# kirilllzaitsev/vision_mtl

Measured on AMD Instinct MI355X. Metric: images/sec fwd+bwd, basic model 128x256, higher is better.
Workload: dtype f32

## Files before the change

vision_mtl_amd/csrc/conv_igemm.hip:

```cpp
#include <mutex>
#include <unordered_map>

#include "common.h"

#define BK 32
#define LDT BK

struct ConvP {
  const float* x = nullptr;
  const float* wp = nullptr;
  const float* bias = nullptr;
  float* y = nullptr;
  float* stats = nullptr;
  int B = 0, H = 0, W = 0, Cs = 0;
  int Ho = 0, Wo = 0, ldy = 0;
  int Nw = 0;
  int Cout = 0;
  int KH = 0, KW = 0, stride = 0, pad = 0;
  int Ktot = 0, M = 0;
  int act = 0;
  int shuffle = 0;
  int tiles_m = 0, tiles_n = 0;
  const float* x2 = nullptr;
  int C2s = 0;
  int ksplit = 1, ksteps_per_split = 0;
  const float* ez_x = nullptr;
  const float* ez_mean = nullptr;
  const float* ez_invstd = nullptr;
  const float* ez_gamma = nullptr;
  const float* ez_beta = nullptr;
  int ez_act = 0;
};

__device__ __attribute__((aligned(16))) float g_zero_page[4] = {0.f, 0.f, 0.f, 0.f};

template <int N>
__device__ __forceinline__ void wait_vmcnt() {
  asm volatile("s_waitcnt vmcnt(%0)" ::"n"(N) : "memory");
}

__device__ __forceinline__ void glds16(const float* src, float* lds_dst) {
  __builtin_amdgcn_global_load_lds((const __attribute__((address_space(1))) void*)src,
                                   (__attribute__((address_space(3))) void*)lds_dst, 16, 0, 0);
}


__device__ __forceinline__ void split3(f32x4 v, u32x2& p1, u32x2& p2, u32x2& p3) {
  unsigned x[4], r1[4], r2[4];
#pragma unroll
  for (int e = 0; e < 4; ++e) {
    x[e] = __float_as_uint(v[e]);
    const float f1 = v[e] - __uint_as_float(x[e] & 0xFFFF0000u);
    r1[e] = __float_as_uint(f1);
    const float f2 = f1 - __uint_as_float(r1[e] & 0xFFFF0000u);
    r2[e] = __float_as_uint(f2);
  }
  p1 = (u32x2){__builtin_amdgcn_perm(x[1], x[0], 0x07060302u), __builtin_amdgcn_perm(x[3], x[2], 0x07060302u)};
  p2 = (u32x2){__builtin_amdgcn_perm(r1[1], r1[0], 0x07060302u), __builtin_amdgcn_perm(r1[3], r1[2], 0x07060302u)};
  p3 = (u32x2){__builtin_amdgcn_perm(r2[1], r2[0], 0x07060302u), __builtin_amdgcn_perm(r2[3], r2[2], 0x07060302u)};
}

template <int TM, int TN, int WAVES_M, int WAVES_N, bool UP2 = false, int NT = 0, int NS = 0, int PL = 0>
__global__ __launch_bounds__(256, (TM * TN >= 20 && WAVES_N == 2) ? 2 : 1) void conv_igemm_kernel(ConvP p) {
  constexpr int BM = WAVES_M * TM * 16;
  constexpr int BNM = WAVES_N * TN * 16;
  constexpr int BN = BNM + NT;
  constexpr int RA = (BM + 31) / 32;
  constexpr int RB = (BN + 31) / 32;
  constexpr int NBUF = NS >= 2 ? NS : 2;
  constexpr int BNR = NS >= 2 ? RB * 32 : BN;
  static_assert(WAVES_M * WAVES_N == 4, "4 waves per workgroup");
  static_assert(NT == 0 || WAVES_N == 1, "tail columns need all waves to span the full tile width");
  static_assert(NS == 0 || (NS >= 2 && NS <= 4 && BM % 32 == 0), "LDS-DMA staging: 2..4 buffers, whole 32-row passes");
  static_assert(PL == 0 || PL == 1 || PL == 3, "operand planes: fp32, bf16 or bf16x3");
  static_assert(PL == 0 || (NS == 0 && (NT == 0 || PL == 1)), "bf16 operands: register staging; bf16x3: no tail columns");

  extern __shared__ __attribute__((aligned(16))) float smem[];
  float* As = smem;
  float* Bs = smem + NBUF * BM * LDT;

  const int tid = threadIdx.x;
  const int lane = tid & 63;
  const int wv = tid >> 6;
  const int wm = wv / WAVES_N, wn = wv % WAVES_N;
  const int l15 = lane & 15, lq = lane >> 4;

  const int nwg = p.tiles_m * p.tiles_n;
  const int bid = xcd_remap(blockIdx.x, nwg);
  const int tile_m = bid / p.tiles_n, tile_n = bid % p.tiles_n;
  const int n0 = tile_n * BN;
  const int tiles_q = UP2 ? p.tiles_m >> 2 : p.tiles_m;
  const int phase = UP2 ? tile_m / tiles_q : 0;
  const int pa = phase >> 1, pb = phase & 1;
  const int m0 = (UP2 ? tile_m - phase * tiles_q : tile_m) * BM;
  const float* wp = p.wp + (UP2 ? (size_t)phase * p.Nw * p.Ktot : 0);

  const int r0 = tid >> 3;
  const int k4 = NS >= 2 ? ((tid & 7) ^ (r0 & 7)) : (tid & 7);
  int pixbase[RA], hb[RA], wb[RA];
  int lb, lho, lwo;
  {
    const int hw = p.Ho * p.Wo, m = m0 + r0;
    lb = m / hw;
    const int rem = m - lb * hw;
    lho = rem / p.Wo;
    lwo = rem - lho * p.Wo;
  }
#pragma unroll
  for (int i = 0; i < RA; ++i) {
    const int m = m0 + r0 + 32 * i;
    if (i > 0) {
      lwo += 32;
      while (lwo >= p.Wo) {
        lwo -= p.Wo;
        if (++lho == p.Ho) {
          lho = 0;
          ++lb;
        }
      }
    }
    if (r0 + 32 * i < BM && m < p.M) {
      const int b = lb, ho = lho, wo = lwo;
      pixbase[i] = b * p.H * p.W;
      hb[i] = UP2 ? ho - 1 + pa : ho * p.stride - p.pad;
      wb[i] = UP2 ? wo - 1 + pb : wo * p.stride - p.pad;
    } else {
      pixbase[i] = 0;
      hb[i] = -(1 << 20);
      wb[i] = 0;
    }
  }
  int kk = k4 * 4;
  int seg = 0, dh = 0, dw = 0, ci = kk;
  int cseg = p.Cs, kwseg = UP2 ? 2 : p.KW;
  auto normalize = [&]() {
    while (ci >= cseg) {
      ci -= cseg;
      if (++dw == kwseg) {
        dw = 0;
        ++dh;
        if (UP2 && seg == 0 && dh == 2) {
          if (p.C2s == 0) { dh = 1 << 20; break; }
          seg = 1; dh = 0; cseg = p.C2s; kwseg = 3;
        }
      }
    }
  };
  normalize();

  f32x4 ra[RA], rb[RB];

  const __amdgpu_buffer_rsrc_t rs_x = buf_rsrc(p.x, (int)((unsigned)p.B * p.H * p.W * p.Cs * 4u));
  const __amdgpu_buffer_rsrc_t rs_x2 =
      buf_rsrc(UP2 && p.x2 != nullptr ? p.x2 : p.x, UP2 ? (int)(16u * p.B * p.H * p.W * p.C2s) : 0);
  const __amdgpu_buffer_rsrc_t rs_w = buf_rsrc(wp, (int)((unsigned)p.Nw * p.Ktot * 4u));
  constexpr unsigned OOB = 0xFFFFFFFFu;
  auto bload = [](__amdgpu_buffer_rsrc_t r, unsigned off) -> f32x4 {
    return __builtin_bit_cast(f32x4, __builtin_amdgcn_raw_buffer_load_b128(r, off, 0, 0));
  };

  int kchunk = 0;
  unsigned rowb0[RA], rowb1[RA];
#pragma unroll
  for (int i = 0; i < RA; ++i) {
    rowb0[i] = (unsigned)(pixbase[i] + hb[i] * p.W + wb[i]) * (unsigned)p.Cs * 4u;
    rowb1[i] = UP2 ? (unsigned)(4 * pixbase[i] + (2 * hb[i] + 1 - pa) * (2 * p.W) + (2 * wb[i] + 1 - pb)) *
                         (unsigned)p.C2s * 4u
                   : 0u;
  }
  unsigned wrowb[RB];
  bool wrow_ok[RB];
#pragma unroll
  for (int i = 0; i < RB; ++i) {
    const int n = n0 + r0 + 32 * i;
    wrow_ok[i] = n < p.Nw && r0 + 32 * i < BN;
    wrowb[i] = (unsigned)n * (unsigned)p.Ktot * 4u;
  }
  auto load_a_seg0 = [&](int i, bool kok, unsigned tapb) {
    const int h = hb[i] + dh, w = wb[i] + dw;
    const bool ok = kok && (unsigned)h < (unsigned)p.H && (unsigned)w < (unsigned)p.W;
    ra[i] = bload(rs_x, ok ? rowb0[i] + tapb : OOB);
  };
  auto load_a_seg1 = [&](int i, bool kok, unsigned tapb) {
    const int h = 2 * hb[i] + 1 - pa + dh, w = 2 * wb[i] + 1 - pb + dw;
    const bool ok = kok && (unsigned)h < (unsigned)(2 * p.H) && (unsigned)w < (unsigned)(2 * p.W);
    ra[i] = bload(rs_x2, ok ? rowb1[i] + tapb : OOB);
  };
  auto load_tile = [&]() {
    const bool kok = kk < p.Ktot;
    const int seg_end = 4 * p.Cs;
    const unsigned tap0 = ((unsigned)(dh * p.W + dw) * (unsigned)p.Cs + (unsigned)ci) * 4u;
    if (!UP2 || kchunk + BK <= seg_end || p.C2s == 0) {
#pragma unroll
      for (int i = 0; i < RA; ++i) load_a_seg0(i, kok && (!UP2 || seg == 0), tap0);
    } else {
      const unsigned tap1 = ((unsigned)(dh * (2 * p.W) + dw) * (unsigned)p.C2s + (unsigned)ci) * 4u;
      if (kchunk >= seg_end) {
#pragma unroll
        for (int i = 0; i < RA; ++i) load_a_seg1(i, kok, tap1);
      } else {
#pragma unroll
        for (int i = 0; i < RA; ++i) {
          if (seg == 0) load_a_seg0(i, kok, tap0);
          else load_a_seg1(i, kok, tap1);
        }
      }
    }
#pragma unroll
    for (int i = 0; i < RB; ++i) rb[i] = bload(rs_w, (kok && wrow_ok[i]) ? wrowb[i] + (unsigned)kk * 4u : OOB);
    kchunk += BK;
    kk += BK;
    ci += BK;
    normalize();
  };
  unsigned char* A3 = reinterpret_cast<unsigned char*>(smem);
  unsigned char* B3 = A3 + 2 * (PL ? PL : 1) * BM * 64;
  auto store_tile = [&](int buf) {
    if constexpr (PL == 1) {
#pragma unroll
      for (int i = 0; i < RA; ++i) {
        const int row = r0 + 32 * i;
        if (BM % 32 == 0 || row < BM)
          *reinterpret_cast<u32x2*>(A3 + (buf * BM + row) * 64 + (((k4 >> 1) ^ ((row >> 2) & 3)) << 4) + ((k4 & 1) << 3)) =
              round_bf16x4(ra[i]);
      }
#pragma unroll
      for (int i = 0; i < RB; ++i) {
        const int row = r0 + 32 * i;
        if (BN % 32 == 0 || row < BN)
          *reinterpret_cast<u32x2*>(B3 + (buf * BN + row) * 64 + (((k4 >> 1) ^ ((row >> 2) & 3)) << 4) + ((k4 & 1) << 3)) =
              round_bf16x4(rb[i]);
      }
      return;
    }
    if constexpr (PL == 3) {
#pragma unroll
      for (int i = 0; i < RA; ++i) {
        const int row = r0 + 32 * i;
        if (BM % 32 == 0 || row < BM) {
          const int off = row * 64 + (((k4 >> 1) ^ ((row >> 2) & 3)) << 4) + ((k4 & 1) << 3);
          u32x2 p1, p2, p3;
          split3(ra[i], p1, p2, p3);
          *reinterpret_cast<u32x2*>(A3 + ((buf * 3 + 0) * BM) * 64 + off) = p1;
          *reinterpret_cast<u32x2*>(A3 + ((buf * 3 + 1) * BM) * 64 + off) = p2;
          *reinterpret_cast<u32x2*>(A3 + ((buf * 3 + 2) * BM) * 64 + off) = p3;
        }
      }
#pragma unroll
      for (int i = 0; i < RB; ++i) {
        const int row = r0 + 32 * i;
        if (BN % 32 == 0 || row < BN) {
          const int off = row * 64 + (((k4 >> 1) ^ ((row >> 2) & 3)) << 4) + ((k4 & 1) << 3);
          u32x2 p1, p2, p3;
          split3(rb[i], p1, p2, p3);
          *reinterpret_cast<u32x2*>(B3 + ((buf * 3 + 0) * BN) * 64 + off) = p1;
          *reinterpret_cast<u32x2*>(B3 + ((buf * 3 + 1) * BN) * 64 + off) = p2;
          *reinterpret_cast<u32x2*>(B3 + ((buf * 3 + 2) * BN) * 64 + off) = p3;
        }
      }
      return;
    }
    float* a = As + buf * BM * LDT;
    float* b = Bs + buf * BNR * LDT;
    const int ks = (k4 ^ (r0 & 7)) * 4;
#pragma unroll
    for (int i = 0; i < RA; ++i)
      if (BM % 32 == 0 || r0 + 32 * i < BM) *reinterpret_cast<f32x4*>(a + (r0 + 32 * i) * LDT + ks) = ra[i];
#pragma unroll
    for (int i = 0; i < RB; ++i)
      if (BN % 32 == 0 || r0 + 32 * i < BN) *reinterpret_cast<f32x4*>(b + (r0 + 32 * i) * LDT + ks) = rb[i];
  };

  f32x4 acc[TM][TN];
#pragma unroll
  for (int i = 0; i < TM; ++i)
#pragma unroll
    for (int j = 0; j < TN; ++j) acc[i][j] = (f32x4){0.f, 0.f, 0.f, 0.f};
  f32x2 tacc[TM][NT > 0 ? NT : 1];
#pragma unroll
  for (int i = 0; i < TM; ++i)
#pragma unroll
    for (int t = 0; t < (NT > 0 ? NT : 1); ++t) tacc[i][t] = (f32x2){0.f, 0.f};

  int nk = (p.Ktot + BK - 1) / BK;
  if (p.ksplit > 1) {
    const int k_begin = blockIdx.y * p.ksteps_per_split;
    nk = min(nk - k_begin, p.ksteps_per_split);
    kk += k_begin * BK;
    ci += k_begin * BK;
    kchunk += k_begin * BK;
    normalize();
  }
  const int ntc = NT > 0 ? max(0, min(NT, p.Nw - (n0 + BNM))) : 0;
  auto compute = [&](int cur) {
    if constexpr (PL == 1) {
      bf16x8 fa[TM];
#pragma unroll
      for (int i = 0; i < TM; ++i) {
        const int row = (wm * TM + i) * 16 + l15;
        fa[i] = *reinterpret_cast<const bf16x8*>(A3 + (cur * BM + row) * 64 + ((lq ^ ((row >> 2) & 3)) << 4));
      }
#pragma unroll
      for (int j = 0; j < TN; ++j) {
        const int row = (wn * TN + j) * 16 + l15;
        const bf16x8 fb = *reinterpret_cast<const bf16x8*>(B3 + (cur * BN + row) * 64 + ((lq ^ ((row >> 2) & 3)) << 4));
#pragma unroll
        for (int i = 0; i < TM; ++i) acc[i][j] = __builtin_amdgcn_mfma_f32_16x16x32_bf16(fa[i], fb, acc[i][j], 0, 0, 0);
      }
      if (NT > 0) {
#pragma unroll
        for (int t = 0; t < NT; ++t) {
          if (t >= ntc) break;
          const int row = BNM + t;
          const bf16x8 ft = *reinterpret_cast<const bf16x8*>(B3 + (cur * BN + row) * 64 + ((lq ^ ((row >> 2) & 3)) << 4));
#pragma unroll
          for (int i = 0; i < TM; ++i)
#pragma unroll
            for (int e = 0; e < 8; e += 2)
              tacc[i][t] += (f32x2){(float)fa[i][e], (float)fa[i][e + 1]} * (f32x2){(float)ft[e], (float)ft[e + 1]};
        }
      }
      return;
    }
    if constexpr (PL == 3) {
      bf16x8 fa[TM][3];
#pragma unroll
      for (int i = 0; i < TM; ++i) {
        const int row = (wm * TM + i) * 16 + l15;
        const int off = row * 64 + ((lq ^ ((row >> 2) & 3)) << 4);
#pragma unroll
        for (int s3 = 0; s3 < 3; ++s3) fa[i][s3] = *reinterpret_cast<const bf16x8*>(A3 + ((cur * 3 + s3) * BM) * 64 + off);
      }
#pragma unroll
      for (int j = 0; j < TN; ++j) {
        const int row = (wn * TN + j) * 16 + l15;
        const int off = row * 64 + ((lq ^ ((row >> 2) & 3)) << 4);
        bf16x8 fb[3];
#pragma unroll
        for (int s3 = 0; s3 < 3; ++s3) fb[s3] = *reinterpret_cast<const bf16x8*>(B3 + ((cur * 3 + s3) * BN) * 64 + off);
#pragma unroll
        for (int i = 0; i < TM; ++i) {
          f32x4 c = acc[i][j];
          c = __builtin_amdgcn_mfma_f32_16x16x32_bf16(fa[i][2], fb[0], c, 0, 0, 0);
          c = __builtin_amdgcn_mfma_f32_16x16x32_bf16(fa[i][1], fb[1], c, 0, 0, 0);
          c = __builtin_amdgcn_mfma_f32_16x16x32_bf16(fa[i][0], fb[2], c, 0, 0, 0);
          c = __builtin_amdgcn_mfma_f32_16x16x32_bf16(fa[i][1], fb[0], c, 0, 0, 0);
          c = __builtin_amdgcn_mfma_f32_16x16x32_bf16(fa[i][0], fb[1], c, 0, 0, 0);
          c = __builtin_amdgcn_mfma_f32_16x16x32_bf16(fa[i][0], fb[0], c, 0, 0, 0);
          acc[i][j] = c;
        }
      }
      return;
    }
    const float* a = As + cur * BM * LDT + (wm * TM * 16 + l15) * LDT;
    const float* b = Bs + cur * BNR * LDT + (wn * TN * 16 + l15) * LDT;
#pragma unroll
    for (int kg = 0; kg < BK / 16; ++kg) {
      const int so = ((kg * 4 + lq) ^ (l15 & 7)) * 4;
      f32x4 fa[TM], fb[TN];
#pragma unroll
      for (int i = 0; i < TM; ++i) fa[i] = *reinterpret_cast<const f32x4*>(a + i * 16 * LDT + so);
#pragma unroll
      for (int j = 0; j < TN; ++j) fb[j] = *reinterpret_cast<const f32x4*>(b + j * 16 * LDT + so);
#ifdef VMTL_SETPRIO
      __builtin_amdgcn_s_setprio(1);
#endif
#pragma unroll
      for (int e = 0; e < 4; ++e)
#pragma unroll
        for (int i = 0; i < TM; ++i)
#pragma unroll
          for (int j = 0; j < TN; ++j)
            acc[i][j] = __builtin_amdgcn_mfma_f32_16x16x4f32(fa[i][e], fb[j][e], acc[i][j], 0, 0, 0);
#ifdef VMTL_SETPRIO
      __builtin_amdgcn_s_setprio(0);
#endif
      if (NT > 0) {
#pragma unroll
        for (int t = 0; t < NT; ++t) {
          if (t >= ntc) break;
          const f32x4 ft = *reinterpret_cast<const f32x4*>(Bs + cur * BNR * LDT + (BNM + t) * LDT +
                                                           (((kg * 4 + lq) ^ ((BNM + t) & 7)) * 4));
          const f32x2 ft_lo = __builtin_shufflevector(ft, ft, 0, 1), ft_hi = __builtin_shufflevector(ft, ft, 2, 3);
#pragma unroll
          for (int i = 0; i < TM; ++i) {
            tacc[i][t] += __builtin_shufflevector(fa[i], fa[i], 0, 1) * ft_lo;
            tacc[i][t] += __builtin_shufflevector(fa[i], fa[i], 2, 3) * ft_hi;
          }
        }
      }
    }
  };

  if constexpr (NS >= 2) {
    constexpr int G = RA + RB;
    auto issue = [&](int buf) {
      const bool kok = kk < p.Ktot;
      float* ad = As + (buf * BM + wv * 8) * LDT;
#pragma unroll
      for (int i = 0; i < RA; ++i) {
        const float* src = g_zero_page;
        if (!UP2 || seg == 0) {
          const int h = hb[i] + dh, w = wb[i] + dw;
          if (kok && (unsigned)h < (unsigned)p.H && (unsigned)w < (unsigned)p.W)
            src = p.x + (size_t)(pixbase[i] + h * p.W + w) * p.Cs + ci;
        } else {
          const int h = 2 * hb[i] + 1 - pa + dh, w = 2 * wb[i] + 1 - pb + dw;
          if (kok && (unsigned)h < (unsigned)(2 * p.H) && (unsigned)w < (unsigned)(2 * p.W))
            src = p.x2 + ((size_t)4 * pixbase[i] + (size_t)h * (2 * p.W) + w) * p.C2s + ci;
        }
        glds16(src, ad + i * 32 * LDT);
      }
      float* bd = Bs + (buf * BNR + wv * 8) * LDT;
#pragma unroll
      for (int i = 0; i < RB; ++i) {
        const int n = n0 + r0 + 32 * i;
        const float* src = g_zero_page;
        if (kok && n < p.Nw && r0 + 32 * i < BN) src = wp + (size_t)n * p.Ktot + kk;
        glds16(src, bd + i * 32 * LDT);
      }
      kk += BK;
      ci += BK;
      normalize();
    };
    int issued = 0;
    for (; issued < NS - 1 && issued < nk; ++issued) issue(issued);
    for (int kt = 0; kt < nk; ++kt) {
      const int pending = issued - kt - 1;
      if (NS >= 4 && pending >= 2) wait_vmcnt<2 * G>();
      else if (NS >= 3 && pending >= 1) wait_vmcnt<G>();
      else wait_vmcnt<0>();
      asm volatile("s_barrier" ::: "memory");
      if (issued < nk) {
        issue(issued % NS);
        ++issued;
      }
      compute(kt % NS);
    }
    __syncthreads();
  } else {
    load_tile();
    store_tile(0);
    __syncthreads();
    int cur = 0;
    for (int kt = 0; kt < nk; ++kt) {
      const bool more = kt + 1 < nk;
      if (more) load_tile();
      compute(cur);
      if (more) store_tile(cur ^ 1);
      __syncthreads();
      cur ^= 1;
    }
  }

  float zs1[TN], zs2[TN];
  if (p.ez_x != nullptr) {
#pragma unroll
    for (int j = 0; j < TN; ++j) {
      const int n = n0 + (wn * TN + j) * 16 + l15;
      const bool nok = n < p.Cout;
      const float em = nok ? p.ez_mean[n] : 0.f, ei = nok ? p.ez_invstd[n] : 0.f;
      const float eg = nok ? p.ez_gamma[n] : 0.f, eb = nok ? p.ez_beta[n] : 0.f;
      float a1 = 0.f, a2 = 0.f;
#pragma unroll
      for (int i = 0; i < TM; ++i)
#pragma unroll
        for (int r = 0; r < 4; ++r) {
          const int m = m0 + (wm * TM + i) * 16 + 4 * lq + r;
          float v = 0.f;
          if (nok && m < p.M) {
            const float xh = (p.ez_x[(size_t)m * p.ldy + n] - em) * ei;
            v = acc[i][j][r] * act_grad(eg * xh + eb, p.ez_act);
            a1 += v;
            a2 += v * xh;
          }
          acc[i][j][r] = v;
        }
      zs1[j] = a1;
      zs2[j] = a2;
    }
  }

  const int hw = p.Ho * p.Wo;
  float* yout = p.ksplit > 1 ? p.y + (size_t)blockIdx.y * (UP2 ? 4 : 1) * p.M * p.ldy : p.y;
  size_t up2_off[TM][4];
  if (UP2 || p.shuffle) {
    const int mb = m0 + wm * TM * 16 + 4 * lq;
    const int b0 = mb / hw, rem0 = mb - b0 * hw;
    const int h0 = rem0 / p.Wo, w0 = rem0 - h0 * p.Wo;
#pragma unroll
    for (int i = 0; i < TM; ++i)
#pragma unroll
      for (int r = 0; r < 4; ++r) {
        int w_ = w0 + i * 16 + r, h_ = h0, b_ = b0;
        while (w_ >= p.Wo) {
          w_ -= p.Wo;
          if (++h_ == p.Ho) {
            h_ = 0;
            ++b_;
          }
        }
        up2_off[i][r] = ((size_t)(b_ * 2 * p.Ho + 2 * h_ + pa) * (2 * p.Wo) + 2 * w_ + pb) * p.ldy;
      }
  }
  float bv[TN];
#pragma unroll
  for (int j = 0; j < TN; ++j) {
    const int n = n0 + (wn * TN + j) * 16 + l15;
    int shco = n;
    size_t shuf_off = 0;
    if (p.shuffle) {
      const int shq = n / p.Cout;
      shco = n - shq * p.Cout;
      shuf_off = ((size_t)(shq >> 1) * (2 * p.Wo) + (shq & 1)) * p.ldy + shco;
    }
    bv[j] = (p.bias != nullptr && n < p.Nw) ? p.bias[p.shuffle ? shco : n] : 0.f;
#pragma unroll
    for (int i = 0; i < TM; ++i) {
#pragma unroll
      for (int r = 0; r < 4; ++r) {
        const int m = m0 + (wm * TM + i) * 16 + 4 * lq + r;
        if (m >= p.M) continue;
        float v = act_fwd(acc[i][j][r] + bv[j], p.act);
        if (UP2) {
          if (n < p.ldy) {
            if (n >= p.Cout) v = 0.f;
            yout[up2_off[i][r] + n] = v;
          }
        } else if (!p.shuffle) {
          if (n < p.ldy) {
            if (n >= p.Cout) v = 0.f;
            yout[(size_t)m * p.ldy + n] = v;
          }
        } else if (n < p.Nw) {
          p.y[up2_off[i][r] + shuf_off] = v;
        }
      }
    }
  }

  float tv[TM][NT > 0 ? NT : 1], txh[TM][NT > 0 ? NT : 1];
  size_t up2_tail_off[(UP2 && NT > 0) ? TM : 1];
  if (UP2 && NT > 0) {
    const int mb = m0 + wm * TM * 16 + l15;
    const int b0 = mb / hw, rem0 = mb - b0 * hw;
    const int h0 = rem0 / p.Wo, w0 = rem0 - h0 * p.Wo;
#pragma unroll
    for (int i = 0; i < TM; ++i) {
      int w_ = w0 + i * 16, h_ = h0, b_ = b0;
      while (w_ >= p.Wo) {
        w_ -= p.Wo;
        if (++h_ == p.Ho) {
          h_ = 0;
          ++b_;
        }
      }
      up2_tail_off[i] = ((size_t)(b_ * 2 * p.Ho + 2 * h_ + pa) * (2 * p.Wo) + 2 * w_ + pb) * p.ldy;
    }
  }
  if (NT > 0) {
#pragma unroll
    for (int i = 0; i < TM; ++i)
#pragma unroll
      for (int t = 0; t < NT; ++t) {
        float v = quarter_sum(tacc[i][t][0] + tacc[i][t][1]);
        const int n = n0 + BNM + t;
        const int m = m0 + (wm * TM + i) * 16 + l15;
        const float bt = (p.bias != nullptr && n < p.Nw) ? p.bias[n] : 0.f;
        v = (n < p.Cout) ? act_fwd(v + bt, p.act) : 0.f;
        if (p.ez_x != nullptr) {
          float xh = 0.f;
          if (n < p.Cout && m < p.M) {
            xh = (p.ez_x[(size_t)m * p.ldy + n] - p.ez_mean[n]) * p.ez_invstd[n];
            v *= act_grad(p.ez_gamma[n] * xh + p.ez_beta[n], p.ez_act);
          } else {
            v = 0.f;
          }
          txh[i][t] = xh;
        }
        tv[i][t] = v;
        if (lq == 0 && m < p.M && n < p.ldy) {
          if (UP2) {
            yout[up2_tail_off[i] + n] = v;
          } else {
            yout[(size_t)m * p.ldy + n] = v;
          }
        }
      }
  }

  if (p.stats != nullptr && p.ez_x != nullptr) {
    float* red = smem;
#pragma unroll
    for (int j = 0; j < TN; ++j) {
      float a1 = zs1[j], a2 = zs2[j];
      a1 = quarter_sum(a1);
      a2 = quarter_sum(a2);
      if (lq == 0) {
        red[wm * BN + (wn * TN + j) * 16 + l15] = a1;
        red[(WAVES_M + wm) * BN + (wn * TN + j) * 16 + l15] = a2;
      }
    }
    if (NT > 0) {
#pragma unroll
      for (int t = 0; t < NT; ++t) {
        float a1 = 0.f, a2 = 0.f;
#pragma unroll
        for (int i = 0; i < TM; ++i) {
          a1 += tv[i][t];
          a2 += tv[i][t] * txh[i][t];
        }
#pragma unroll
        for (int o = 1; o < 16; o <<= 1) {
          a1 += __shfl_xor(a1, o, 64);
          a2 += __shfl_xor(a2, o, 64);
        }
        if (lane == 0) {
          red[wm * BN + BNM + t] = a1;
          red[(WAVES_M + wm) * BN + BNM + t] = a2;
        }
      }
    }
    __syncthreads();
    for (int c = tid; c < BN; c += 256) {
      float a1 = 0.f, a2 = 0.f;
#pragma unroll
      for (int w = 0; w < WAVES_M; ++w) {
        a1 += red[w * BN + c];
        a2 += red[(WAVES_M + w) * BN + c];
      }
      const int n = n0 + c;
      if (n < p.ldy) {
        p.stats[((size_t)tile_m * 2 + 0) * p.ldy + n] = a1;
        p.stats[((size_t)tile_m * 2 + 1) * p.ldy + n] = a2;
      }
    }
  } else if (p.stats != nullptr) {
    float* red = smem;
    const int nvalid = min(BM, p.M - m0);
    auto colval = [&](int i, int j, int r, float& v) -> bool {
      const int m = m0 + (wm * TM + i) * 16 + 4 * lq + r;
      const int n = n0 + (wn * TN + j) * 16 + l15;
      v = (n < p.Cout) ? act_fwd(acc[i][j][r] + bv[j], p.act) : 0.f;
      return m < p.M;
    };
#pragma unroll
    for (int j = 0; j < TN; ++j) {
      float v0;
      colval(0, j, 0, v0);
      const float pv = quarter0_bcast(v0);
      float s1 = 0.f, s2 = 0.f;
#pragma unroll
      for (int i = 0; i < TM; ++i)
#pragma unroll
        for (int r = 0; r < 4; ++r) {
          float v;
          if (colval(i, j, r, v)) {
            const float d = v - pv;
            s1 += d;
            s2 += d * d;
          }
        }
      s1 = quarter_sum(s1);
      s2 = quarter_sum(s2);
      if (lq == 0) {
        const int c = (wn * TN + j) * 16 + l15;
        red[(0 * WAVES_M + wm) * BN + c] = s1;
        red[(1 * WAVES_M + wm) * BN + c] = s2;
        red[(2 * WAVES_M + wm) * BN + c] = pv;
      }
    }
    if (NT > 0) {
#pragma unroll
      for (int t = 0; t < NT; ++t) {
        const float pv = __shfl(tv[0][t], 0, 64);
        float s1 = 0.f, s2 = 0.f;
#pragma unroll
        for (int i = 0; i < TM; ++i)
          if (m0 + (wm * TM + i) * 16 + l15 < p.M) {
            const float d = tv[i][t] - pv;
            s1 += d;
            s2 += d * d;
          }
#pragma unroll
        for (int o = 1; o < 16; o <<= 1) {
          s1 += __shfl_xor(s1, o, 64);
          s2 += __shfl_xor(s2, o, 64);
        }
        if (lane == 0) {
          red[(0 * WAVES_M + wm) * BN + BNM + t] = s1;
          red[(1 * WAVES_M + wm) * BN + BNM + t] = s2;
          red[(2 * WAVES_M + wm) * BN + BNM + t] = pv;
        }
      }
    }
    __syncthreads();
    if (nvalid == BM) {
      constexpr float inv_n = 1.f / (TM * 16), inv_w = 1.f / WAVES_M;
      for (int c = tid; c < BN; c += 256) {
        float mw[WAVES_M], mean = 0.f, m2 = 0.f;
#pragma unroll
        for (int w = 0; w < WAVES_M; ++w) {
          const float s1 = red[(0 * WAVES_M + w) * BN + c], s2 = red[(1 * WAVES_M + w) * BN + c];
          mw[w] = red[(2 * WAVES_M + w) * BN + c] + s1 * inv_n;
          m2 += s2 - s1 * s1 * inv_n;
          mean += mw[w];
        }
        mean *= inv_w;
#pragma unroll
        for (int w = 0; w < WAVES_M; ++w) m2 += (TM * 16) * (mw[w] - mean) * (mw[w] - mean);
        const int n = n0 + c;
        if (n < p.ldy) {
          p.stats[((size_t)tile_m * 2 + 0) * p.ldy + n] = mean;
          p.stats[((size_t)tile_m * 2 + 1) * p.ldy + n] = m2;
        }
      }
      return;
    }
    for (int c = tid; c < BN; c += 256) {
      float cn = 0.f, mean = 0.f, m2 = 0.f;
#pragma unroll
      for (int w = 0; w < WAVES_M; ++w) {
        const float nw = (float)max(0, min(TM * 16, nvalid - w * TM * 16));
        if (nw > 0.f) {
          const float s1 = red[(0 * WAVES_M + w) * BN + c], s2 = red[(1 * WAVES_M + w) * BN + c];
          const float mw = red[(2 * WAVES_M + w) * BN + c] + s1 / nw;
          const float qw = s2 - s1 * s1 / nw;
          const float tot = cn + nw, d = mw - mean;
          mean += d * (nw / tot);
          m2 += qw + d * d * (cn * nw / tot);
          cn = tot;
        }
      }
      const int n = n0 + c;
      if (n < p.ldy) {
        p.stats[((size_t)tile_m * 2 + 0) * p.ldy + n] = mean;
        p.stats[((size_t)tile_m * 2 + 1) * p.ldy + n] = m2;
      }
    }
  }
}

static bool conv_bf16x3() {
  static EnvInt e{"VMTL_BF16X3", 0};
  return env_int(e) == 1;
}

static int conv_glds_stages() {
  static EnvInt e{"VMTL_GLDS", 0};
  const int v = env_int(e);
  return (v == 2 || v == 3) ? v : 0;
}

template <int TM, int TN, int WMV, int WNV, bool UP2, int NT, int NS, int PL = 0>
static int launch_conv_ns(ConvP& p, hipStream_t st) {
  constexpr int BM = WMV * TM * 16, BN = WNV * TN * 16 + NT;
  p.tiles_m = cdiv(p.M, BM) * (UP2 ? 4 : 1);
  p.tiles_n = cdiv(p.shuffle ? p.Nw : p.ldy, BN);
  if ((long long)p.B * p.H * p.W * p.Cs * 4 >= (1ll << 32) || (long long)p.Nw * p.Ktot * 4 >= (1ll << 32) ||
      (UP2 && (long long)16 * p.B * p.H * p.W * p.C2s >= (1ll << 32)))
    return VMTL_ERR_UNSUPPORTED;
  constexpr int NBUF = NS >= 2 ? NS : 2;
  constexpr int BNR = NS >= 2 ? (BN + 31) / 32 * 32 : BN;
  const size_t lds = PL ? (size_t)2 * PL * (BM + BN) * 64 : (size_t)NBUF * (BM + BNR) * LDT * sizeof(float);
  const int rc = allow_dynamic_lds(reinterpret_cast<const void*>(&conv_igemm_kernel<TM, TN, WMV, WNV, UP2, NT, NS, PL>), lds);
  if (rc) return rc;
  hipLaunchKernelGGL((conv_igemm_kernel<TM, TN, WMV, WNV, UP2, NT, NS, PL>),
                     dim3(p.tiles_m * p.tiles_n, p.ksplit > 1 ? p.ksplit : 1), dim3(256), lds, st, p);
  return vmtl_check_launch();
}

template <int TM, int TN, int WMV, int WNV, bool UP2, int NT>
static int launch_conv(ConvP& p, hipStream_t st, int prec) {
  if (prec == VMTL_PREC_BF16) return launch_conv_ns<TM, TN, WMV, WNV, UP2, NT, 0, 1>(p, st);
  if constexpr (NT == 0 && WNV * TN >= 5) {
    if (conv_bf16x3() && cdiv(p.Ktot, BK) >= 24) return launch_conv_ns<TM, TN, WMV, WNV, UP2, NT, 0, 3>(p, st);
  }
  if constexpr (!UP2 && (WMV * TM) % 2 == 0) {
    const int ns = conv_glds_stages();
    if (ns == 2) return launch_conv_ns<TM, TN, WMV, WNV, UP2, NT, 2>(p, st);
    if (ns == 3) return launch_conv_ns<TM, TN, WMV, WNV, UP2, NT, 3>(p, st);
  }
  return launch_conv_ns<TM, TN, WMV, WNV, UP2, NT, 0>(p, st);
}

#define VMTL_CONV_TILES(X)                      \
  X(0, 2, 2, 4, 1, 0, 0.62f)    \
  X(1, 2, 3, 4, 1, 0, 0.72f)    \
  X(2, 2, 4, 4, 1, 0, 0.80f)    \
  X(3, 2, 5, 4, 1, 0, 0.88f)    \
  X(4, 4, 3, 2, 2, 0, 0.92f)    \
  X(5, 4, 4, 2, 2, 0, 0.95f)    \
  X(6, 2, 9, 4, 1, 0, 1.0f)     \
  X(7, 4, 5, 2, 2, 0, 1.0f)     \
  X(8, 1, 2, 4, 1, 0, 0.50f)    \
  X(9, 1, 4, 4, 1, 0, 0.85f)    \
  X(10, 2, 4, 2, 2, 0, 0.75f)   \
  X(11, 1, 9, 4, 1, 0, 1.0f)    \
  X(12, 2, 2, 4, 1, 4, 0.62f)   \
  X(13, 2, 1, 4, 1, 4, 0.43f)   \
  X(14, 2, 4, 4, 1, 4, 0.85f)   \
  X(15, 2, 1, 4, 1, 0, 0.38f)

struct TileCfg { int id, bm, bn; float eff; };
#define VMTL_TILE_CFG(id, TM, TN, WMV, WNV, NT, eff) {id, WMV * TM * 16, WNV * TN * 16 + NT, eff},
static constexpr TileCfg kTiles[] = {VMTL_CONV_TILES(VMTL_TILE_CFG)};
#undef VMTL_TILE_CFG
#define VMTL_NTILES 16
#define VMTL_NBIG 12
static const int kBigIds[] = {0, 1, 2, 3, 4, 5, 6, 7, 12, 13, 14, 15};
static const int kSmallIds[] = {8, 9, 10, 11};

static constexpr bool tiles_in_id_order() {
  for (int i = 0; i < VMTL_NTILES; ++i)
    if (kTiles[i].id != i) return false;
  return true;
}
static_assert(sizeof(kTiles) / sizeof(kTiles[0]) == VMTL_NTILES && tiles_in_id_order(), "kTiles[] is indexed by tile id");

template <bool UP2>
static int launch_tile(int id, ConvP& p, hipStream_t st, int prec) {
  switch (id) {
#define VMTL_TILE_CASE(id, TM, TN, WMV, WNV, NT, eff) \
  case id: return launch_conv<TM, TN, WMV, WNV, UP2, NT>(p, st, prec);
    VMTL_CONV_TILES(VMTL_TILE_CASE)
#undef VMTL_TILE_CASE
    default: return launch_tile<UP2>(VMTL_NTILES - 1, p, st, prec);
  }
}

static int pick_from(const int* ids, int n, int ncols) {
  int best = ids[0];
  float best_cost = -1.f;
  for (int k = 0; k < n; ++k) {
    const int id = ids[k];
    const float cost = (float)((long long)cdiv(ncols, kTiles[id].bn) * kTiles[id].bn) / kTiles[id].eff;
    if (best_cost < 0.f || cost < best_cost) {
      best = id;
      best_cost = cost;
    }
  }
  return best;
}

static int forced_tile() {
  static EnvInt e{"VMTL_FORCE_TILE", -1};
  const int id = env_int(e);
  return (id >= 0 && id < VMTL_NTILES) ? id : -1;
}

static int conv_pick_tile(int M, int ncols) {
  const int forced = forced_tile();
  if (forced >= 0) return forced;
  const int big = pick_from(kBigIds, VMTL_NBIG, ncols);
  if ((long long)cdiv(M, 128) * cdiv(ncols, kTiles[big].bn) < 384) return pick_from(kSmallIds, 4, ncols);
  if (conv_bf16x3() && kTiles[big].bn >= 80) return pick_from(kSmallIds, 4, ncols);
  return big;
}

extern "C" int vmtl_conv2d_stats_rows(int B, int Ho, int Wo, int ldy) {
  return cdiv(B * Ho * Wo, kTiles[conv_pick_tile(B * Ho * Wo, ldy)].bm);
}

extern "C" int vmtl_conv2d_stats_block(int B, int Ho, int Wo, int ldy) {
  return kTiles[conv_pick_tile(B * Ho * Wo, ldy)].bm;
}

__global__ __launch_bounds__(256) void sum_slabs_kernel(const float* __restrict__ slabs, float* __restrict__ y,
                                                        int nslabs, long long n4, const float* __restrict__ bias,
                                                        int ldy, int Cout) {
  VMTL_GRID_STRIDE(i, n4) {
    f32x4 s = reinterpret_cast<const f32x4*>(slabs)[i];
    for (int z = 1; z < nslabs; ++z) s += reinterpret_cast<const f32x4*>(slabs)[(size_t)z * n4 + i];
    if (bias != nullptr) {
      const int n = (int)((i * 4) % ldy);
#pragma unroll
      for (int e = 0; e < 4; ++e)
        if (n + e < Cout) s[e] += bias[n + e];
    }
    reinterpret_cast<f32x4*>(y)[i] = s;
  }
}

static int ksplit_for(long long blocks, int nk, int ldy) {
  static EnvInt e_blocks{"VMTL_KSPLIT_BLOCKS", 512};
  const int target = env_int(e_blocks);
  if (blocks <= 0 || blocks >= target || nk < 32 || (ldy & 3)) return 1;
  long long s = cdivll(target, blocks);
  if (s > 8) s = 8;
  if (s > nk / 16) s = nk / 16;
  return s < 2 ? 1 : (int)s;
}

template <bool UP2>
static int launch_split(int id, ConvP& p, int splits, float* ws, float* y, const float* bias, hipStream_t st, int prec) {
  p.y = ws;
  p.ksplit = splits;
  p.ksteps_per_split = cdiv(cdiv(p.Ktot, BK), splits);
  const int rc = launch_tile<UP2>(id, p, st, prec);
  if (rc) return rc;
  const long long n4 = (long long)(UP2 ? 4 : 1) * p.M * p.ldy / 4;
  hipLaunchKernelGGL(sum_slabs_kernel, dim3(grid_1d(n4, 256, 4096)), dim3(256), 0, st, ws, y, splits, n4, bias, p.ldy,
                     p.Cout);
  return vmtl_check_launch();
}

extern "C" int vmtl_conv2d_ksplit(int B, int Ho, int Wo, int ldy, int Ktot) {
  if (B <= 0 || Ho <= 0 || Wo <= 0 || ldy <= 0 || Ktot <= 0) return 1;
  const int M = B * Ho * Wo;
  const int id = conv_pick_tile(M, ldy);
  return ksplit_for((long long)cdiv(M, kTiles[id].bm) * cdiv(ldy, kTiles[id].bn), cdiv(Ktot, BK), ldy);
}

static int conv2d_check(const float* x, const float* wp, const float* y, const float* stats, int B, int H, int W, int Cs,
                        int Ho, int Wo, int ldy, int Nw, int Cout, int KH, int KW, int stride, int pad, int shuffle) {
  if (!x || !wp || !y) return VMTL_ERR_ARG;
  if (Cs <= 0 || (Cs & 3) || B <= 0 || H <= 0 || W <= 0 || Ho <= 0 || Wo <= 0) return VMTL_ERR_ARG;
  if (KH <= 0 || KW <= 0 || stride <= 0 || pad < 0 || Nw <= 0 || Cout <= 0 || ldy <= 0) return VMTL_ERR_ARG;
  if (!shuffle && (Cout > ldy || Nw > ldy)) return VMTL_ERR_ARG;
  if (shuffle && (Nw != 4 * Cout || Cout > ldy || stats)) return VMTL_ERR_ARG;
  if ((H + 2 * pad - KH) / stride + 1 != Ho || (W + 2 * pad - KW) / stride + 1 != Wo) return VMTL_ERR_ARG;
  if ((long long)B * Ho * Wo > 0x7fffffffLL || (long long)B * H * W > 0x7fffffffLL) return VMTL_ERR_ARG;
  return VMTL_OK;
}

static ConvP conv2d_params(const float* x, const float* wp, float* y, int B, int H, int W, int Cs, int Ho, int Wo,
                           int ldy, int Nw, int Cout, int KH, int KW, int stride, int pad) {
  ConvP p;
  p.x = x; p.wp = wp; p.y = y;
  p.B = B; p.H = H; p.W = W; p.Cs = Cs; p.Ho = Ho; p.Wo = Wo; p.ldy = ldy; p.Nw = Nw; p.Cout = Cout;
  p.KH = KH; p.KW = KW; p.stride = stride; p.pad = pad; p.Ktot = KH * KW * Cs; p.M = B * Ho * Wo;
  return p;
}

static int conv2d_fwd_impl(const float* x, const float* wp, const float* bias, float* y, float* stats,
                           int B, int H, int W, int Cs, int Ho, int Wo, int ldy, int Nw, int Cout,
                           int KH, int KW, int stride, int pad, int act, int shuffle, const float* ez_x,
                           const float* ez_mean, const float* ez_invstd, const float* ez_gamma, const float* ez_beta,
                           int ez_act, int prec, void* stream) {
  VMTL_ENTER();
  if (!valid_prec(prec)) return VMTL_ERR_ARG;
  if (conv2d_check(x, wp, y, stats, B, H, W, Cs, Ho, Wo, ldy, Nw, Cout, KH, KW, stride, pad, shuffle)) return VMTL_ERR_ARG;
  ConvP p = conv2d_params(x, wp, y, B, H, W, Cs, Ho, Wo, ldy, Nw, Cout, KH, KW, stride, pad);
  p.bias = bias; p.stats = stats; p.act = act; p.shuffle = shuffle;
  p.ez_x = ez_x; p.ez_mean = ez_mean; p.ez_invstd = ez_invstd; p.ez_gamma = ez_gamma; p.ez_beta = ez_beta; p.ez_act = ez_act;
  hipStream_t st = (hipStream_t)stream;
  if (shuffle && ldy > Cout &&
      hipMemsetAsync(y, 0, (size_t)B * 4 * Ho * Wo * ldy * sizeof(float), st) != hipSuccess)
    return VMTL_ERR_LAUNCH;
  return launch_tile<false>(conv_pick_tile(p.M, shuffle ? Nw : ldy), p, st, prec);
}

extern "C" int vmtl_conv2d_fwd_p(const float* x, const float* wp, const float* bias, float* y, float* stats,
                                 int B, int H, int W, int Cs, int Ho, int Wo, int ldy, int Nw, int Cout,
                                 int KH, int KW, int stride, int pad, int act, int shuffle, int precision, void* stream) {
  return conv2d_fwd_impl(x, wp, bias, y, stats, B, H, W, Cs, Ho, Wo, ldy, Nw, Cout, KH, KW, stride, pad, act, shuffle,
                         nullptr, nullptr, nullptr, nullptr, nullptr, 0, precision, stream);
}

extern "C" int vmtl_conv2d_fwd(const float* x, const float* wp, const float* bias, float* y, float* stats,
                               int B, int H, int W, int Cs, int Ho, int Wo, int ldy, int Nw, int Cout,
                               int KH, int KW, int stride, int pad, int act, int shuffle, void* stream) {
  return vmtl_conv2d_fwd_p(x, wp, bias, y, stats, B, H, W, Cs, Ho, Wo, ldy, Nw, Cout, KH, KW, stride, pad, act, shuffle,
                           VMTL_PREC_FP32, stream);
}

extern "C" int vmtl_conv2d_bnbwd_p(const float* x, const float* wp, float* y, float* stats, const float* ez_x,
                                   const float* ez_mean, const float* ez_invstd, const float* ez_gamma,
                                   const float* ez_beta, int ez_act, int B, int H, int W, int Cs, int Ho, int Wo, int ldy,
                                   int Nw, int Cout, int KH, int KW, int stride, int pad, int precision, void* stream) {
  if (!valid_prec(precision) || !stats || !ez_x || !ez_mean || !ez_invstd || !ez_gamma || !ez_beta) return VMTL_ERR_ARG;
  return conv2d_fwd_impl(x, wp, nullptr, y, stats, B, H, W, Cs, Ho, Wo, ldy, Nw, Cout, KH, KW, stride, pad, 0, 0, ez_x,
                         ez_mean, ez_invstd, ez_gamma, ez_beta, ez_act, precision, stream);
}

extern "C" int vmtl_conv2d_bnbwd(const float* x, const float* wp, float* y, float* stats, const float* ez_x,
                                 const float* ez_mean, const float* ez_invstd, const float* ez_gamma,
                                 const float* ez_beta, int ez_act, int B, int H, int W, int Cs, int Ho, int Wo, int ldy,
                                 int Nw, int Cout, int KH, int KW, int stride, int pad, void* stream) {
  return vmtl_conv2d_bnbwd_p(x, wp, y, stats, ez_x, ez_mean, ez_invstd, ez_gamma, ez_beta, ez_act, B, H, W, Cs, Ho, Wo, ldy,
                             Nw, Cout, KH, KW, stride, pad, VMTL_PREC_FP32, stream);
}

extern "C" int vmtl_conv2d_fwd_ws_p(const float* x, const float* wp, const float* bias, float* y, float* ws, int B, int H,
                                    int W, int Cs, int Ho, int Wo, int ldy, int Nw, int Cout, int KH, int KW, int stride,
                                    int pad, int precision, void* stream) {
  VMTL_ENTER();
  if (!valid_prec(precision)) return VMTL_ERR_ARG;
  if (conv2d_check(x, wp, y, nullptr, B, H, W, Cs, Ho, Wo, ldy, Nw, Cout, KH, KW, stride, pad, 0)) return VMTL_ERR_ARG;
  const int splits = vmtl_conv2d_ksplit(B, Ho, Wo, ldy, KH * KW * Cs);
  if (splits <= 1 || ws == nullptr)
    return vmtl_conv2d_fwd_p(x, wp, bias, y, nullptr, B, H, W, Cs, Ho, Wo, ldy, Nw, Cout, KH, KW, stride, pad, 0, 0,
                             precision, stream);
  ConvP p = conv2d_params(x, wp, y, B, H, W, Cs, Ho, Wo, ldy, Nw, Cout, KH, KW, stride, pad);
  return launch_split<false>(conv_pick_tile(p.M, ldy), p, splits, ws, y, bias, (hipStream_t)stream, precision);
}

extern "C" int vmtl_conv2d_fwd_ws(const float* x, const float* wp, const float* bias, float* y, float* ws, int B, int H,
                                  int W, int Cs, int Ho, int Wo, int ldy, int Nw, int Cout, int KH, int KW, int stride,
                                  int pad, void* stream) {
  return vmtl_conv2d_fwd_ws_p(x, wp, bias, y, ws, B, H, W, Cs, Ho, Wo, ldy, Nw, Cout, KH, KW, stride, pad, VMTL_PREC_FP32,
                              stream);
}

static int up2_pick_tile(int Mq, int ncols) {
  const int forced = forced_tile();
  if (forced >= 0) return forced;
  int big = pick_from(kBigIds, VMTL_NBIG, ncols);
  if (big == 14) big = 3;
  if ((long long)cdiv(Mq, 128) * 4 * cdiv(ncols, kTiles[big].bn) < 384) return pick_from(kSmallIds, 4, ncols);
  if (conv_bf16x3() && kTiles[big].bn >= 80) return pick_from(kSmallIds, 4, ncols);
  return big;
}

extern "C" int vmtl_conv2d_up2_stats_block(int B, int H2, int W2, int ldy) {
  return kTiles[up2_pick_tile(B * H2 * W2, ldy)].bm;
}

extern "C" int vmtl_conv2d_up2_ksplit(int B, int H2, int W2, int ldy, int Ktot) {
  if (B <= 0 || H2 <= 0 || W2 <= 0 || ldy <= 0 || Ktot <= 0) return 1;
  const int Mq = B * H2 * W2;
  const int id = up2_pick_tile(Mq, ldy);
  return ksplit_for((long long)cdiv(Mq, kTiles[id].bm) * 4 * cdiv(ldy, kTiles[id].bn), cdiv(Ktot, BK), ldy);
}

static int up2_check(const float* xl, const float* skip, const float* wp_eff, const float* y, int B, int H2, int W2,
                     int C0s, int C1s, int ldy, int Cout) {
  if (!xl || !wp_eff || !y || B <= 0 || H2 <= 0 || W2 <= 0 || C0s <= 0 || (C0s & 3) || (C1s & 3) || C1s < 0)
    return VMTL_ERR_ARG;
  if ((skip == nullptr) != (C1s == 0) || Cout <= 0 || Cout > ldy || (ldy & 3)) return VMTL_ERR_ARG;
  if ((long long)B * H2 * W2 * 4 > 0x7fffffffLL) return VMTL_ERR_ARG;
  return VMTL_OK;
}

static ConvP up2_params(const float* xl, const float* skip, const float* wp_eff, float* y, int B, int H2, int W2, int C0s,
                        int C1s, int ldy, int Cout) {
  ConvP p;
  p.x = xl; p.x2 = skip; p.wp = wp_eff; p.y = y;
  p.B = B; p.H = H2; p.W = W2; p.Cs = C0s; p.C2s = C1s; p.Ho = H2; p.Wo = W2; p.ldy = ldy; p.Nw = Cout;
  p.Cout = Cout; p.KH = 2; p.KW = 2; p.stride = 1; p.pad = 0; p.Ktot = 4 * C0s + 9 * C1s; p.M = B * H2 * W2;
  return p;
}

extern "C" int vmtl_conv2d_up2_fwd_p(const float* xl, const float* skip, const float* wp_eff, float* y, float* stats,
                                     int B, int H2, int W2, int C0s, int C1s, int ldy, int Cout, int precision,
                                     void* stream) {
  VMTL_ENTER();
  if (!valid_prec(precision)) return VMTL_ERR_ARG;
  if (up2_check(xl, skip, wp_eff, y, B, H2, W2, C0s, C1s, ldy, Cout)) return VMTL_ERR_ARG;
  ConvP p = up2_params(xl, skip, wp_eff, y, B, H2, W2, C0s, C1s, ldy, Cout);
  p.stats = stats;
  const int id = up2_pick_tile(p.M, ldy);
  if (stats && (p.M % kTiles[id].bm)) return VMTL_ERR_ARG;
  return launch_tile<true>(id, p, (hipStream_t)stream, precision);
}

extern "C" int vmtl_conv2d_up2_fwd(const float* xl, const float* skip, const float* wp_eff, float* y, float* stats,
                                   int B, int H2, int W2, int C0s, int C1s, int ldy, int Cout, void* stream) {
  return vmtl_conv2d_up2_fwd_p(xl, skip, wp_eff, y, stats, B, H2, W2, C0s, C1s, ldy, Cout, VMTL_PREC_FP32, stream);
}

extern "C" int vmtl_conv2d_up2_fwd_ws_p(const float* xl, const float* skip, const float* wp_eff, float* y, float* ws,
                                        int B, int H2, int W2, int C0s, int C1s, int ldy, int Cout, int precision,
                                        void* stream) {
  VMTL_ENTER();
  if (!valid_prec(precision)) return VMTL_ERR_ARG;
  if (up2_check(xl, skip, wp_eff, y, B, H2, W2, C0s, C1s, ldy, Cout)) return VMTL_ERR_ARG;
  const int splits = vmtl_conv2d_up2_ksplit(B, H2, W2, ldy, 4 * C0s + 9 * C1s);
  if (splits <= 1 || ws == nullptr)
    return vmtl_conv2d_up2_fwd_p(xl, skip, wp_eff, y, nullptr, B, H2, W2, C0s, C1s, ldy, Cout, precision, stream);
  ConvP p = up2_params(xl, skip, wp_eff, y, B, H2, W2, C0s, C1s, ldy, Cout);
  return launch_split<true>(up2_pick_tile(p.M, ldy), p, splits, ws, y, nullptr, (hipStream_t)stream, precision);
}

extern "C" int vmtl_conv2d_up2_fwd_ws(const float* xl, const float* skip, const float* wp_eff, float* y, float* ws, int B,
                                      int H2, int W2, int C0s, int C1s, int ldy, int Cout, void* stream) {
  return vmtl_conv2d_up2_fwd_ws_p(xl, skip, wp_eff, y, ws, B, H2, W2, C0s, C1s, ldy, Cout, VMTL_PREC_FP32, stream);
}
```

Baseline: 2740.

## Add software-pipelined fragment reads to fp32 implicit-GEMM conv main loop

Adds a PP=1 kernel variant that reads the first k-group's LDS fragments before issuing the next tile's global loads, so the global-load latency overlaps MFMA work, with a sched_barrier to keep that ordering. It is enabled by default through an env switch for tile configs flagged in a new per-tile column. The tail-column epilogue also gains handling for shuffle (pixel-shuffle) output addressing and bias indexing. Holding the prefetched fragments across the load raises register pressure, which may reduce occupancy.

```diff
diff --git a/vision_mtl_amd/csrc/conv_igemm.hip b/vision_mtl_amd/csrc/conv_igemm.hip
--- a/vision_mtl_amd/csrc/conv_igemm.hip
+++ b/vision_mtl_amd/csrc/conv_igemm.hip
@@ -60,7 +60,7 @@
   p3 = (u32x2){__builtin_amdgcn_perm(r2[1], r2[0], 0x07060302u), __builtin_amdgcn_perm(r2[3], r2[2], 0x07060302u)};
 }
 
-template <int TM, int TN, int WAVES_M, int WAVES_N, bool UP2 = false, int NT = 0, int NS = 0, int PL = 0>
+template <int TM, int TN, int WAVES_M, int WAVES_N, bool UP2 = false, int NT = 0, int NS = 0, int PL = 0, int PP = 0>
 __global__ __launch_bounds__(256, (TM * TN >= 20 && WAVES_N == 2) ? 2 : 1) void conv_igemm_kernel(ConvP p) {
   constexpr int BM = WAVES_M * TM * 16;
   constexpr int BNM = WAVES_N * TN * 16;
@@ -74,6 +74,7 @@
   static_assert(NS == 0 || (NS >= 2 && NS <= 4 && BM % 32 == 0), "LDS-DMA staging: 2..4 buffers, whole 32-row passes");
   static_assert(PL == 0 || PL == 1 || PL == 3, "operand planes: fp32, bf16 or bf16x3");
   static_assert(PL == 0 || (NS == 0 && (NT == 0 || PL == 1)), "bf16 operands: register staging; bf16x3: no tail columns");
+  static_assert(PP == 0 || (PP == 1 && NS == 0 && PL == 0), "pipelined fragment reads: the fp32 register-staging loop");
 
   extern __shared__ __attribute__((aligned(16))) float smem[];
   float* As = smem;
@@ -392,7 +393,61 @@
     }
   };
 
-  if constexpr (NS >= 2) {
+  f32x4 pfa[TM], pfb[TN];
+  auto read_frags = [&](int cur, int kg, f32x4(&fa)[TM], f32x4(&fb)[TN]) {
+    const float* a = As + cur * BM * LDT + (wm * TM * 16 + l15) * LDT;
+    const float* b = Bs + cur * BNR * LDT + (wn * TN * 16 + l15) * LDT;
+    const int so = ((kg * 4 + lq) ^ (l15 & 7)) * 4;
+#pragma unroll
+    for (int i = 0; i < TM; ++i) fa[i] = *reinterpret_cast<const f32x4*>(a + i * 16 * LDT + so);
+#pragma unroll
+    for (int j = 0; j < TN; ++j) fb[j] = *reinterpret_cast<const f32x4*>(b + j * 16 * LDT + so);
+  };
+  auto mfma_kgroup = [&](int cur, int kg, const f32x4(&fa)[TM], const f32x4(&fb)[TN]) {
+#pragma unroll
+    for (int e = 0; e < 4; ++e)
+#pragma unroll
+      for (int i = 0; i < TM; ++i)
+#pragma unroll
+        for (int j = 0; j < TN; ++j)
+          acc[i][j] = __builtin_amdgcn_mfma_f32_16x16x4f32(fa[i][e], fb[j][e], acc[i][j], 0, 0, 0);
+    if (NT > 0) {
+#pragma unroll
+      for (int t = 0; t < NT; ++t) {
+        if (t >= ntc) break;
+        const f32x4 ft = *reinterpret_cast<const f32x4*>(Bs + cur * BNR * LDT + (BNM + t) * LDT +
+                                                         (((kg * 4 + lq) ^ ((BNM + t) & 7)) * 4));
+        const f32x2 ft_lo = __builtin_shufflevector(ft, ft, 0, 1), ft_hi = __builtin_shufflevector(ft, ft, 2, 3);
+#pragma unroll
+        for (int i = 0; i < TM; ++i) {
+          tacc[i][t] += __builtin_shufflevector(fa[i], fa[i], 0, 1) * ft_lo;
+          tacc[i][t] += __builtin_shufflevector(fa[i], fa[i], 2, 3) * ft_hi;
+        }
+      }
+    }
+  };
+
+  if constexpr (PP == 1) {
+    load_tile();
+    store_tile(0);
+    __syncthreads();
+    int cur = 0;
+    for (int kt = 0; kt < nk; ++kt) {
+      const bool more = kt + 1 < nk;
+      read_frags(cur, 0, pfa, pfb);
+      __builtin_amdgcn_sched_barrier(0);
+      if (more) load_tile();
+      mfma_kgroup(cur, 0, pfa, pfb);
+      {
+        f32x4 fa[TM], fb[TN];
+        read_frags(cur, 1, fa, fb);
+        mfma_kgroup(cur, 1, fa, fb);
+      }
+      if (more) store_tile(cur ^ 1);
+      __syncthreads();
+      cur ^= 1;
+    }
+  } else if constexpr (NS >= 2) {
     constexpr int G = RA + RB;
     auto issue = [&](int buf) {
       const bool kok = kk < p.Ktot;
@@ -566,8 +621,14 @@
         float v = quarter_sum(tacc[i][t][0] + tacc[i][t][1]);
         const int n = n0 + BNM + t;
         const int m = m0 + (wm * TM + i) * 16 + l15;
-        const float bt = (p.bias != nullptr && n < p.Nw) ? p.bias[n] : 0.f;
-        v = (n < p.Cout) ? act_fwd(v + bt, p.act) : 0.f;
+        const bool sh = !UP2 && p.shuffle;
+        int shq = 0, shco = n;
+        if (sh) {
+          shq = n / p.Cout;
+          shco = n - shq * p.Cout;
+        }
+        const float bt = (p.bias != nullptr && n < p.Nw) ? p.bias[shco] : 0.f;
+        v = (n < (sh ? p.Nw : p.Cout)) ? act_fwd(v + bt, p.act) : 0.f;
         if (p.ez_x != nullptr) {
           float xh = 0.f;
           if (n < p.Cout && m < p.M) {
@@ -579,7 +640,13 @@
           txh[i][t] = xh;
         }
         tv[i][t] = v;
-        if (lq == 0 && m < p.M && n < p.ldy) {
+        if (sh) {
+          if (lq == 0 && m < p.M && n < p.Nw) {
+            const int b_ = m / hw, rem_ = m - b_ * hw;
+            const int h_ = rem_ / p.Wo, w_ = rem_ - h_ * p.Wo;
+            p.y[((size_t)(b_ * 2 * p.Ho + 2 * h_ + (shq >> 1)) * (2 * p.Wo) + 2 * w_ + (shq & 1)) * p.ldy + shco] = v;
+          }
+        } else if (lq == 0 && m < p.M && n < p.ldy) {
           if (UP2) {
             yout[up2_tail_off[i] + n] = v;
           } else {
@@ -752,7 +819,7 @@
   return (v == 2 || v == 3) ? v : 0;
 }
 
-template <int TM, int TN, int WMV, int WNV, bool UP2, int NT, int NS, int PL = 0>
+template <int TM, int TN, int WMV, int WNV, bool UP2, int NT, int NS, int PL = 0, int PP = 0>
 static int launch_conv_ns(ConvP& p, hipStream_t st) {
   constexpr int BM = WMV * TM * 16, BN = WNV * TN * 16 + NT;
   p.tiles_m = cdiv(p.M, BM) * (UP2 ? 4 : 1);
@@ -763,15 +830,21 @@
   constexpr int NBUF = NS >= 2 ? NS : 2;
   constexpr int BNR = NS >= 2 ? (BN + 31) / 32 * 32 : BN;
   const size_t lds = PL ? (size_t)2 * PL * (BM + BN) * 64 : (size_t)NBUF * (BM + BNR) * LDT * sizeof(float);
-  const int rc = allow_dynamic_lds(reinterpret_cast<const void*>(&conv_igemm_kernel<TM, TN, WMV, WNV, UP2, NT, NS, PL>), lds);
+  const int rc = allow_dynamic_lds(reinterpret_cast<const void*>(&conv_igemm_kernel<TM, TN, WMV, WNV, UP2, NT, NS, PL, PP>), lds);
   if (rc) return rc;
-  hipLaunchKernelGGL((conv_igemm_kernel<TM, TN, WMV, WNV, UP2, NT, NS, PL>),
+  hipLaunchKernelGGL((conv_igemm_kernel<TM, TN, WMV, WNV, UP2, NT, NS, PL, PP>),
                      dim3(p.tiles_m * p.tiles_n, p.ksplit > 1 ? p.ksplit : 1), dim3(256), lds, st, p);
   return vmtl_check_launch();
 }
 
+static bool conv_igemm_pipe(int tile_default) {
+  static EnvInt e{"VMTL_IGEMM_PIPE", 1};
+  const int v = env_int(e);
+  return v == 2 || (v == 1 && tile_default != 0);
+}
+
 template <int TM, int TN, int WMV, int WNV, bool UP2, int NT>
-static int launch_conv(ConvP& p, hipStream_t st, int prec) {
+static int launch_conv(ConvP& p, hipStream_t st, int prec, int pipe) {
   if (prec == VMTL_PREC_BF16) return launch_conv_ns<TM, TN, WMV, WNV, UP2, NT, 0, 1>(p, st);
   if constexpr (NT == 0 && WNV * TN >= 5) {
     if (conv_bf16x3() && cdiv(p.Ktot, BK) >= 24) return launch_conv_ns<TM, TN, WMV, WNV, UP2, NT, 0, 3>(p, st);
@@ -781,29 +854,30 @@
     if (ns == 2) return launch_conv_ns<TM, TN, WMV, WNV, UP2, NT, 2>(p, st);
     if (ns == 3) return launch_conv_ns<TM, TN, WMV, WNV, UP2, NT, 3>(p, st);
   }
+  if (conv_igemm_pipe(pipe)) return launch_conv_ns<TM, TN, WMV, WNV, UP2, NT, 0, 0, 1>(p, st);
   return launch_conv_ns<TM, TN, WMV, WNV, UP2, NT, 0>(p, st);
 }
 
 #define VMTL_CONV_TILES(X)                      \
-  X(0, 2, 2, 4, 1, 0, 0.62f)    \
-  X(1, 2, 3, 4, 1, 0, 0.72f)    \
-  X(2, 2, 4, 4, 1, 0, 0.80f)    \
-  X(3, 2, 5, 4, 1, 0, 0.88f)    \
-  X(4, 4, 3, 2, 2, 0, 0.92f)    \
-  X(5, 4, 4, 2, 2, 0, 0.95f)    \
-  X(6, 2, 9, 4, 1, 0, 1.0f)     \
-  X(7, 4, 5, 2, 2, 0, 1.0f)     \
-  X(8, 1, 2, 4, 1, 0, 0.50f)    \
-  X(9, 1, 4, 4, 1, 0, 0.85f)    \
-  X(10, 2, 4, 2, 2, 0, 0.75f)   \
-  X(11, 1, 9, 4, 1, 0, 1.0f)    \
-  X(12, 2, 2, 4, 1, 4, 0.62f)   \
-  X(13, 2, 1, 4, 1, 4, 0.43f)   \
-  X(14, 2, 4, 4, 1, 4, 0.85f)   \
-  X(15, 2, 1, 4, 1, 0, 0.38f)
+  X(0, 2, 2, 4, 1, 0, 0.62f, 1)    \
+  X(1, 2, 3, 4, 1, 0, 0.72f, 1)    \
+  X(2, 2, 4, 4, 1, 0, 0.80f, 1)    \
+  X(3, 2, 5, 4, 1, 0, 0.88f, 0)    \
+  X(4, 4, 3, 2, 2, 0, 0.92f, 0)    \
+  X(5, 4, 4, 2, 2, 0, 0.95f, 1)    \
+  X(6, 2, 9, 4, 1, 0, 1.0f, 1)     \
+  X(7, 4, 5, 2, 2, 0, 1.0f, 1)     \
+  X(8, 1, 2, 4, 1, 0, 0.50f, 1)    \
+  X(9, 1, 4, 4, 1, 0, 0.85f, 1)    \
+  X(10, 2, 4, 2, 2, 0, 0.75f, 1)   \
+  X(11, 1, 9, 4, 1, 0, 1.0f, 1)    \
+  X(12, 2, 2, 4, 1, 4, 0.62f, 0)   \
+  X(13, 2, 1, 4, 1, 4, 0.43f, 0)   \
+  X(14, 2, 4, 4, 1, 4, 0.85f, 0)   \
+  X(15, 2, 1, 4, 1, 0, 0.38f, 0)
 
 struct TileCfg { int id, bm, bn; float eff; };
-#define VMTL_TILE_CFG(id, TM, TN, WMV, WNV, NT, eff) {id, WMV * TM * 16, WNV * TN * 16 + NT, eff},
+#define VMTL_TILE_CFG(id, TM, TN, WMV, WNV, NT, eff, pipe) {id, WMV * TM * 16, WNV * TN * 16 + NT, eff},
 static constexpr TileCfg kTiles[] = {VMTL_CONV_TILES(VMTL_TILE_CFG)};
 #undef VMTL_TILE_CFG
 #define VMTL_NTILES 16
@@ -821,8 +895,8 @@
 template <bool UP2>
 static int launch_tile(int id, ConvP& p, hipStream_t st, int prec) {
   switch (id) {
-#define VMTL_TILE_CASE(id, TM, TN, WMV, WNV, NT, eff) \
-  case id: return launch_conv<TM, TN, WMV, WNV, UP2, NT>(p, st, prec);
+#define VMTL_TILE_CASE(id, TM, TN, WMV, WNV, NT, eff, pipe) \
+  case id: return launch_conv<TM, TN, WMV, WNV, UP2, NT>(p, st, prec, pipe);
     VMTL_CONV_TILES(VMTL_TILE_CASE)
 #undef VMTL_TILE_CASE
     default: return launch_tile<UP2>(VMTL_NTILES - 1, p, st, prec);
```

After: 2747 (median of 6 runs). Within noise of the previous version (+0.3%).
